# chilir/spotter

Measured on AMD Instinct MI355X. Metric: images/sec RT-DETRv2-R101 640² bs32 at 1/2/4/8 MI355X; p50 /detect latency, higher is better.
Workload: dtype fp32; 1 GPU; RT-DETRv2-r101vd 640x640 batch=32/GPU preprocess+forward+postprocess; model=rtdetr_v2_r101vd, global_batch=32, image_size=640, parallelism=replicas x1

## Files before the change

### include/spotter_hip.h

```cpp
#ifndef SPOTTER_HIP_H
#define SPOTTER_HIP_H

#include <stddef.h>
#include <stdint.h>

#ifdef __cplusplus
extern "C" {
#endif

#define SP_ABI_VERSION 20

enum sp_act { SP_ACT_NONE = 0, SP_ACT_RELU = 1, SP_ACT_SILU = 2, SP_ACT_GELU = 3 };
enum sp_precision { SP_PREC_FP32 = 0, SP_PREC_BF16 = 1, SP_PREC_F32X3 = 2, SP_PREC_F32X2 = 3 };

typedef struct {
  const uint8_t* data;
  int32_t height, width;
  int32_t row_stride;
} sp_image_u8;

typedef struct {
  const float* A; int64_t lda;
  const float* A2; int64_t lda2;
  int32_t N, H, W, Cin;
// ... 72 lines not shown
} sp_conv_plan_info;
int sp_conv_plan(const sp_conv_desc* d, sp_conv_plan_info* out);
int sp_set_plan_batch(int batch, int plan_batch);

int sp_conv3x3_winograd(const sp_conv_desc* d, const uint16_t* wt_wino, int64_t wino_plane_stride, float* work,
                        int64_t work_elems, void* stream);
int sp_winograd_f23_input(const sp_conv_desc* d, float* work, int64_t work_elems, void* stream);
int sp_winograd_f23_gemm(const sp_conv_desc* d, const uint16_t* wt_wino, int64_t wino_plane_stride, float* work,
                         int64_t work_elems, void* stream);
int sp_winograd_f23_output(const sp_conv_desc* d, const float* work, int64_t work_elems, void* stream);
int sp_winograd_f43_input(const sp_conv_desc* d, float* work, int64_t work_elems, void* stream);
int sp_winograd_f43_gemm(const sp_conv_desc* d, const uint16_t* wt_wino, int64_t wino_plane_stride, float* work,
                         int64_t work_elems, void* stream);
int sp_winograd_f43_output(const sp_conv_desc* d, const float* work, int64_t work_elems, void* stream);
typedef struct {
  sp_conv_plan_info gemm;
  int32_t components;
  int32_t in_vw;
  int32_t out_vw;
  int64_t tiles;
} sp_winograd_plan_info;
int sp_winograd_plan(const sp_conv_desc* d, int wm, int64_t wino_plane_stride, int64_t work_elems,
                     sp_winograd_plan_info* out);

int sp_nchw_to_nhwc(const float* x, float* y, int n, int c, int h, int w, void* stream);
int sp_stem_conv3x3s2_nchw(const float* x, const float* wt, const float* scale, const float* shift, float* y,
                           int n, int h, int w, int cout, int act, void* stream);
int sp_stem_conv3x3s2_nchw_bf16(const float* x, const float* wt, const float* scale, const float* shift, uint16_t* y,
                                int n, int h, int w, int cout, int act, void* stream);
int sp_conv3x3_c32_bf16(const uint16_t* x, const uint16_t* w16, const float* scale, const float* shift, uint16_t* y,
                        int n, int h, int w, int cout, int act, void* stream);
int sp_conv3x3_c32(const float* x, const float* wt, const float* scale, const float* shift, float* y, int n, int h,
                   int w, int cout, int act, void* stream);
int sp_conv3x3_c64_bf16(const uint16_t* x, int64_t ldx, const uint16_t* w16, const float* scale, const float* shift,
                        uint16_t* y, int64_t ldy, const uint16_t* res, int64_t ldr, int n, int h, int w, int act,
                        void* stream);
int sp_conv3x3_c64_x3(const float* x, int64_t ldx, const uint16_t* w_planes, int64_t plane_stride, const float* scale,
                      const float* shift, float* y, int64_t ldy, int n, int h, int w, int act, void* stream);
int sp_conv3x3_c32_x3(const float* x, const uint16_t* w_planes, int64_t plane_stride, const float* scale,
                      const float* shift, float* y, int n, int h, int w, int cout, int act, void* stream);
int sp_maxpool3x3s2(const float* x, float* y, int64_t ldy, int n, int h, int w, int c, void* stream);
int sp_maxpool3x3s2_bf16(const uint16_t* x, uint16_t* y, int64_t ldy, int n, int h, int w, int c, void* stream);
int sp_avgpool2x2_ceil(const float* x, float* y, int64_t ldy, int n, int h, int w, int c, void* stream);
int sp_avgpool2x2_ceil_bf16(const uint16_t* x, uint16_t* y, int64_t ldy, int n, int h, int w, int c, void* stream);
int sp_upsample2x_nearest(const float* x, int64_t ldx, float* y, int64_t ldy, int n, int h,
                          int w, int c, void* stream);
// ... 117 lines not shown
```

### spotter_amd/_lib.py

```python
from __future__ import annotations

import ctypes as C
import os
import threading

HERE = os.path.dirname(os.path.abspath(__file__))
LIB_PATH = os.environ.get("SPOTTER_HIP_LIB", os.path.join(HERE, "libspotter_hip.so"))
ABI_VERSION = 20

vp = C.c_void_p
i32 = C.c_int32
i64 = C.c_int64
f32 = C.c_float


class SpImageU8(C.Structure):
    _fields_ = [("data", vp), ("height", i32), ("width", i32), ("row_stride", i32)]


class SpConvDesc(C.Structure):
    _fields_ = [
        ("A", vp), ("lda", i64), ("A2", vp), ("lda2", i64),
        ("N", i32), ("H", i32), ("W", i32), ("Cin", i32),
        ("KH", i32), ("KW", i32), ("stride", i32), ("pad", i32),
# ... 2 lines not shown
        ("scale", vp), ("shift", vp),
        ("row_scale", vp), ("row_period", i32),
        ("res1", vp), ("ldr1", i64),
        ("act", i32),
        ("res2", vp), ("ldr2", i64),
        ("C", vp), ("ldc", i64),
        ("out_rows_per_group", i32), ("out_group_stride", i64),
        ("workspace", vp), ("workspace_elems", i64),
        ("precision", i32), ("Wt_bf16", vp), ("wt_plane_stride", i64),
        ("ln_gamma", vp), ("ln_beta", vp), ("ln_eps", f32),
        ("A_bf16", vp),
        ("C_bf16", vp), ("res1_bf16", vp), ("res2_bf16", vp),
        ("splitk_counters", vp), ("splitk_counters_len", i64),
    ]


class SpConvPlanInfo(C.Structure):
    _fields_ = [(f, i32) for f in ("family", "tile", "planes", "generic", "a_bf16", "fast_1x1", "epilogue", "splits",
                                   "counters")]


class SpWinogradPlanInfo(C.Structure):
    _fields_ = [("gemm", SpConvPlanInfo), ("components", i32), ("in_vw", i32), ("out_vw", i32), ("tiles", i64)]


class SpMsdaDesc(C.Structure):
    _fields_ = [
        ("value", vp), ("ld_value", i64), ("value_col", i32),
        ("off_aw", vp), ("ld_off_aw", i64),
        ("ref", vp),
        ("out", vp), ("ld_out", i64),
        ("B", i32), ("S", i32), ("Q", i32), ("heads", i32), ("head_dim", i32),
        ("levels", i32), ("points", i32),
        ("level_h", i32 * 4), ("level_w", i32 * 4), ("level_start", i32 * 4),
        ("offset_scale", f32),
        ("value_bf16", vp),
    ]


class SpJpegLayout(C.Structure):
    _fields_ = [
        ("width", i32), ("height", i32), ("ncomp", i32), ("color", i32), ("progressive", i32),
        ("max_h", i32), ("max_v", i32), ("h", i32 * 3), ("v", i32 * 3), ("bw", i32 * 3), ("bh", i32 * 3),
        ("block_off", i64 * 3), ("total_blocks", i64), ("plane_off", i64 * 3), ("plane_bytes", i64),
        ("quant", (C.c_uint16 * 64) * 3),
    ]
# ... 47 lines not shown

_SIGS = {
    "sp_abi_version": (i32, []),
    "sp_build_flags": (i32, []),
    "sp_bounds_report": (i64, [C.c_char_p, i64]),
    "sp_last_error": (C.c_char_p, []),
    "sp_device_init": (i32, [i32]),
    "sp_shutdown": (i32, []),
    "sp_preprocess_u8": (i32, [C.POINTER(SpImageU8), i32, i32, i32, vp, vp]),
    "sp_conv2d": (i32, [C.POINTER(SpConvDesc), vp]),
    "sp_set_conv_config": (i32, [i32]),
    "sp_set_splitk_config": (i32, [i32, i32, i32]),
    "sp_set_tuning": (i32, [i32, i32]),
    "sp_set_plan_batch": (i32, [i32, i32]),
    "sp_conv_plan": (i32, [C.POINTER(SpConvDesc), C.POINTER(SpConvPlanInfo)]),
    "sp_winograd_plan": (i32, [C.POINTER(SpConvDesc), i32, i64, i64, C.POINTER(SpWinogradPlanInfo)]),
    "sp_conv3x3_winograd": (i32, [C.POINTER(SpConvDesc), vp, i64, vp, i64, vp]),
    "sp_winograd_f23_input": (i32, [C.POINTER(SpConvDesc), vp, i64, vp]),
    "sp_winograd_f23_gemm": (i32, [C.POINTER(SpConvDesc), vp, i64, vp, i64, vp]),
    "sp_winograd_f23_output": (i32, [C.POINTER(SpConvDesc), vp, i64, vp]),
    "sp_winograd_f43_input": (i32, [C.POINTER(SpConvDesc), vp, i64, vp]),
    "sp_winograd_f43_gemm": (i32, [C.POINTER(SpConvDesc), vp, i64, vp, i64, vp]),
    "sp_winograd_f43_output": (i32, [C.POINTER(SpConvDesc), vp, i64, vp]),
    "sp_nchw_to_nhwc": (i32, [vp, vp, i32, i32, i32, i32, vp]),
    "sp_stem_conv3x3s2_nchw": (i32, [vp, vp, vp, vp, vp, i32, i32, i32, i32, i32, vp]),
    "sp_maxpool3x3s2": (i32, [vp, vp, i64, i32, i32, i32, i32, vp]),
    "sp_avgpool2x2_ceil": (i32, [vp, vp, i64, i32, i32, i32, i32, vp]),
    "sp_maxpool3x3s2_bf16": (i32, [vp, vp, i64, i32, i32, i32, i32, vp]),
    "sp_avgpool2x2_ceil_bf16": (i32, [vp, vp, i64, i32, i32, i32, i32, vp]),
    "sp_stem_conv3x3s2_nchw_bf16": (i32, [vp, vp, vp, vp, vp, i32, i32, i32, i32, i32, vp]),
    "sp_conv3x3_c32_bf16": (i32, [vp, vp, vp, vp, vp, i32, i32, i32, i32, i32, vp]),
    "sp_conv3x3_c32": (i32, [vp, vp, vp, vp, vp, i32, i32, i32, i32, i32, vp]),
    "sp_conv3x3_c64_bf16": (i32, [vp, i64, vp, vp, vp, vp, i64, vp, i64, i32, i32, i32, i32, vp]),
    "sp_conv3x3_c64_x3": (i32, [vp, i64, vp, i64, vp, vp, vp, i64, i32, i32, i32, i32, vp]),
    "sp_conv3x3_c32_x3": (i32, [vp, vp, i64, vp, vp, vp, i32, i32, i32, i32, i32, vp]),
    "sp_upsample2x_nearest": (i32, [vp, i64, vp, i64, i32, i32, i32, i32, vp]),
    "sp_layernorm": (i32, [vp, i64, vp, vp, vp, i64, i32, i32, f32, vp]),
    "sp_layernorm_bf16": (i32, [vp, i64, vp, vp, vp, i64, i32, i32, f32, vp]),
    "sp_attention": (i32, [vp, i64, vp, i64, vp, i64, vp, i64, i32, i32, i32, i32, f32, vp]),
    "sp_attention_bf16": (i32, [vp, i64, vp, i64, vp, i64, vp, i64, i32, i32, i32, i32, f32, vp]),
    "sp_msda": (i32, [C.POINTER(SpMsdaDesc), vp]),
    "sp_topk_rows": (i32, [vp, i64, i32, i32, i32, i32, i32, vp, vp, vp]),
    "sp_rowmax": (i32, [vp, i64, i64, i32, vp, vp]),
    "sp_gather_rows": (i32, [vp, i64, i32, vp, i32, i32, i32, vp, i64, vp]),
    "sp_ref_init": (i32, [vp, i64, vp, vp, i32, i32, vp, vp]),
    "sp_box_refine": (i32, [vp, i64, vp, i32, vp]),
# ... 56 lines not shown
```

### spotter_amd/csrc/winograd.hip

```cpp
#include <cstdlib>
#include "conv_plan.h"
#include "mfma16_common.h"

namespace sp {
namespace {

typedef float v4f __attribute__((ext_vector_type(4)));

__device__ __forceinline__ float4 ld_nt(const float* p) {
  const v4f v = __builtin_nontemporal_load(reinterpret_cast<const v4f*>(p));
  return make_float4(v.x, v.y, v.z, v.w);
}

__global__ __launch_bounds__(256) void wino_in_f23_x2_kernel(const float* __restrict__ x, int64_t lda, int h, int w,
                                                             int c4n, int th, int tw, int64_t nb,
                                                             float* __restrict__ V, int64_t cin) {
  const int tw2 = (tw + 1) / 2;
  const int64_t T = nb * th * tw;
  const int64_t total = nb * th * tw2 * c4n;
  const int64_t plane = T * cin;
  for (int64_t g = blockIdx.x * (int64_t)blockDim.x + threadIdx.x; g < total; g += (int64_t)gridDim.x * blockDim.x) {
    const int64_t t2 = g / c4n;
    const int c = (int)(g - t2 * c4n) * 4;
    const int64_t b = t2 / ((int64_t)th * tw2);
// ... 422 lines not shown
    else
      hipLaunchKernelGGL(wino_out_f43_kernel<2>, dim3(stream_grid(T * d->Cout / 2)), dim3(256), 0,
                         as_stream(stream), work + wino_v_floats(NC, T, d->Cin), T, d->Cout / 2, th, tw, *d, ts, cs);
  }
  return check_launch(what);
}

template <int MT>
int wino_plan_info(const sp_conv_desc* d, int64_t wino_plane_stride, int64_t work_elems, sp_winograd_plan_info* out) {
  WinoPlan w;
  if (int rc = wino_plan<MT>("sp_winograd_plan", d, nullptr, wino_plane_stride, nullptr, work_elems, true, false, &w))
    return rc;
  out->gemm = w.p;
  out->components = (MT + 2) * (MT + 2);
  out->in_vw = w.in_vw;
  out->out_vw = w.out_vw;
  out->tiles = w.T;
  return 0;
}

}
}

extern "C" int sp_winograd_f23_input(const sp_conv_desc* d, float* work, int64_t work_elems, void* stream) {
  return sp::wino_input<2>("sp_winograd_f23_input", d, work, work_elems, stream);
}

extern "C" int sp_winograd_f23_gemm(const sp_conv_desc* d, const uint16_t* wt_wino, int64_t wino_plane_stride,
                                    float* work, int64_t work_elems, void* stream) {
  return sp::wino_gemm<2>("sp_winograd_f23_gemm", d, wt_wino, wino_plane_stride, work, work_elems, stream);
}

extern "C" int sp_winograd_f23_output(const sp_conv_desc* d, const float* work, int64_t work_elems, void* stream) {
  return sp::wino_output<2>("sp_winograd_f23_output", d, work, work_elems, stream);
}

extern "C" int sp_conv3x3_winograd(const sp_conv_desc* d, const uint16_t* wt_wino, int64_t wino_plane_stride,
                                   float* work, int64_t work_elems, void* stream) {
  if (int rc = sp_winograd_f23_input(d, work, work_elems, stream)) return rc;
  if (int rc = sp_winograd_f23_gemm(d, wt_wino, wino_plane_stride, work, work_elems, stream)) return rc;
  return sp_winograd_f23_output(d, work, work_elems, stream);
}

extern "C" int sp_winograd_f43_input(const sp_conv_desc* d, float* work, int64_t work_elems, void* stream) {
  return sp::wino_input<4>("sp_winograd_f43_input", d, work, work_elems, stream);
}
// ... 17 lines not shown
```

### spotter_amd/engine.py

```python
from __future__ import annotations

import math

import numpy as np
import torch

from . import ops
from .config import PRECISIONS, SpotterConfig, check_batch_invariant, check_precision
from .ops import V, view
from .weights import backbone_plan


def _t(a, dev):
    return torch.from_numpy(np.ascontiguousarray(a, dtype=np.float32)).to(dev)


bf16_bits = ops.bf16_bits


ATTN_BF16 = True

_X3_FASTER = {(256, 64, False), (256, 1024, True), (1024, 256, True), (512, 256, True), (256, 512, True),
              (288, 256, True), (4, 256, False)}



def _wkw(wq):
    if wq is None:
        return {}
    if wq.dim() == 2 and wq.shape[0] in (2, 3):
        return {"wt_planes": wq}
    return {"wt16": wq}


class ConvW:
    __slots__ = ("w", "cin", "cout", "k", "scale", "shift", "w16", "host", "wino", "mode", "x3p")

    def __init__(self, w, cin, cout, k, scale, shift, w16=None, host=None, mode="f32"):
        self.w, self.cin, self.cout, self.k, self.scale, self.shift = w, cin, cout, k, scale, shift
        self.w16 = w16
        self.mode = mode
        self.host = host
        self.wino = None
        self.x3p = None


class LinW:
    __slots__ = ("w", "b", "k", "n", "w16", "mode")

    def __init__(self, w, b, k, n, w16=None, mode="f32"):
        self.w, self.b, self.k, self.n = w, b, k, n
        self.w16 = w16
        self.mode = mode


def frozen_bn_affine(p, pre):
    scale = p[pre + ".weight"] * (p[pre + ".running_var"] + np.float32(1e-5)) ** np.float32(-0.5)
    shift = p[pre + ".bias"] - p[pre + ".running_mean"] * scale
    return scale.astype(np.float32), shift.astype(np.float32)


def eval_bn_affine(p, pre, eps=1e-5):
    inv = (p[pre + ".running_var"] + np.float32(eps)) ** np.float32(-0.5)
    scale = p[pre + ".weight"] * inv
    shift = p[pre + ".bias"] - p[pre + ".running_mean"] * scale
    return scale.astype(np.float32), shift.astype(np.float32)

# ... 16 lines not shown
    out = []
    f = np.float32
    for lvl, (h, w) in enumerate(shapes):
        gy, gx = np.meshgrid(np.arange(h, dtype=f), np.arange(w, dtype=f), indexing="ij")
        xy = np.stack([gx, gy], -1) + f(0.5)
        xy[..., 0] /= f(w)
        xy[..., 1] /= f(h)
        wh = np.ones_like(xy) * f(grid_size * 2.0 ** lvl)
        out.append(np.concatenate([xy, wh], -1).reshape(h * w, 4))
    a = np.concatenate(out, 0).astype(f)
    valid = ((a > f(1e-2)) & (a < f(1 - 1e-2))).all(-1)
    lg = np.log(a / (f(1) - a)).astype(f)
    lg[~valid] = np.finfo(f).max
    return lg, valid.astype(f)


class Engine:

    def __init__(self, cfg: SpotterConfig, weights: dict, device: str | torch.device = "cuda",
                 fold_repvgg: bool = True, precision: str = "fp32", fuse_shortcut: bool = True,
                 fuse_ln: bool = False, winograd: str | bool = "auto", wino_m: int = 4,
                 bf16_store: bool | None = None, direct_c32: bool = True,
                 direct_c64_bf16: bool = True, splitk_combine: bool = False, direct_c64_x3: bool = True,
                 direct_c32_x3: bool = False, batch_invariant: int | None = None):
        from ._lib import SP_BUILD_FUSED_LN, lib

        check_precision(precision)
        self.batch_invariant = check_batch_invariant(batch_invariant)
        self.cfg = cfg
        self.fold_repvgg = fold_repvgg
        self.fuse_shortcut = fuse_shortcut
        self.fuse_ln = fuse_ln
        if fuse_ln and PRECISIONS.get(precision, ("", ""))[1] == "bf16":
            raise ValueError(f"fuse_ln=True runs the linears on fp32 weights: not available with precision={precision!r}")
        if fuse_ln and not (lib().sp_build_flags() & SP_BUILD_FUSED_LN):
            raise ValueError("fuse_ln=True needs a diagnostic library with the fused-LayerNorm tiles "
                             "(UNIT=conv_gemm tools/build_diag.sh <name> -DSP_DIAG_KERNELS=1; SPOTTER_HIP_LIB)")
        if winograd is True:
            winograd = "auto"
        if winograd not in (False, None, "auto", "repvgg", "all"):
            raise ValueError("winograd must be False, 'auto', 'repvgg' or 'all'")
        self.winograd = winograd or False
        if wino_m not in (2, 4):
            raise ValueError("wino_m must be 2 (F(2x2,3x3)) or 4 (F(4x4,3x3))")
        self.wino_m = wino_m
        self.precision = precision
        self.act_bb = cfg.hidden_act
        self.act_enc = cfg.activation_function
        self.act_aifi = cfg.encoder_activation_function
        self.act_dec = cfg.decoder_activation_function
        self._conv_mode, self._lin_mode = PRECISIONS[precision]
        self._attn_bf16 = self._lin_mode == "bf16" and ATTN_BF16
        self.bf16_store = (self._conv_mode == "bf16") if bf16_store is None else bool(bf16_store)
        if self.bf16_store and self._conv_mode != "bf16":
            raise ValueError("bf16_store needs a bf16 conv operand mode")
        self.direct_c32 = direct_c32
        self.direct_c64_bf16 = direct_c64_bf16
        self.direct_c64_x3 = direct_c64_x3
        self.direct_c32_x3 = direct_c32_x3
        self.splitk_combine = splitk_combine
        self.splitk_min_rows = 0
        self.add_rows = True
        self.enc_head_bf16 = True
        self.enc_rowmax_fused = True
        self.dev = torch.device(device)
        if self.dev.type != "cuda":
            raise RuntimeError("spotter_amd runs on an MI355X (gfx950) device only")
        idx = self.dev.index if self.dev.index is not None else torch.cuda.current_device()
        self.dev = torch.device("cuda", idx)
        rc = lib().sp_device_init(idx)
        if rc != 0:
            raise RuntimeError(f"sp_device_init: {lib().sp_last_error().decode()}")
        with torch.cuda.device(self.dev):
            self._pack(weights)
        self._B = 1
        self._ws = {}
        self._consts = {}
        self._ctxs = {}
        self._outs = {}
        self.microbatches = None
        self.stagger = 1
# ... 58 lines not shown
        cfg = self.cfg
        bb = "model.backbone.model"
        self.stem = [self._conv(p, f"{bb}.embedder.embedder.{i}.convolution.weight",
                                f"{bb}.embedder.embedder.{i}.normalization", True) for i in range(3)]
        if self.precision == "fp32" and self._conv_mode == "x3" and self.direct_c32_x3:
            for cw in self.stem[1:]:
                if cw.cin == 32 and cw.k == 3 and cw.cout in (32, 64) and cw.mode == "f32":
                    cw.x3p = torch.from_numpy(ops.split_bf16x3_host(cw.host)).to(self.dev)
        self.blocks = []
        for (s, i, lt, cin, cout, st, sc) in backbone_plan(cfg):
            pre = f"{bb}.encoder.stages.{s}.layers.{i}"
            blk = {"s": s, "i": i, "type": lt, "cin": cin, "cout": cout, "stride": st, "sc": sc}
            if sc == "conv":
                blk["short"] = self._conv(p, pre + ".shortcut.convolution.weight", pre + ".shortcut.normalization", True)
            elif sc == "avgconv":
                blk["short"] = self._conv(p, pre + ".shortcut.1.convolution.weight", pre + ".shortcut.1.normalization", True)
            nl = 3 if lt == "bottleneck" else 2
            blk["layers"] = [self._conv(p, f"{pre}.layer.{j}.convolution.weight", f"{pre}.layer.{j}.normalization", True)
                             for j in range(nl)]
            if self.winograd in ("auto", "all"):
                for j, c in enumerate(blk["layers"]):
                    if c.k == 3 and (st == 1 or (lt != "bottleneck" and j == 1)):
                        self._add_wino(c)
            if self.fuse_shortcut and lt == "bottleneck" and (sc == "avgconv" or (sc == "conv" and st == 1)):
                sk = pre + (".shortcut.1" if sc == "avgconv" else ".shortcut")
                blk["fused"] = self._fused_tail(p, f"{pre}.layer.2", sk, cin)
            self.blocks.append(blk)
        self.in_proj = [self._conv(p, f"model.encoder_input_proj.{l}.0.weight", f"model.encoder_input_proj.{l}.1", False)
                        for l in range(len(cfg.encoder_in_channels))]
        a = "model.encoder.aifi.0.layers.0"
        self.aifi = {
            "qk": self._lin(p, a + ".self_attn.q_proj", a + ".self_attn.k_proj"),
            "v": self._lin(p, a + ".self_attn.v_proj"),
            "o": self._lin(p, a + ".self_attn.o_proj"),
            "ln1": self._ln(p, a + ".self_attn_layer_norm"),
            "fc1": self._lin(p, a + ".mlp.fc1"),
            "fc2": self._lin(p, a + ".mlp.fc2"),
            "ln2": self._ln(p, a + ".final_layer_norm"),
        }
        E = "model.encoder"
        nl = len(cfg.encoder_in_channels)
        self.lateral = [self._conv(p, f"{E}.lateral_convs.{i}.conv.weight", f"{E}.lateral_convs.{i}.norm", False)
                        for i in range(nl - 1)]
        self.down = [self._conv(p, f"{E}.downsample_convs.{i}.conv.weight", f"{E}.downsample_convs.{i}.norm", False)
                     for i in range(nl - 1)]
        self.fpn = [self._csp(p, f"{E}.fpn_blocks.{i}") for i in range(nl - 1)]
# ... 113 lines not shown
            return pixels * cin >= self.WINO43_MIN_WORK and (cin >= self.WINO43_MIN_CIN or self.winograd != "auto")
        return pixels >= self.WINO_MIN_PIXELS

    def _cv(self, x: V, n, h, w, cw: ConvW, stride, out: V, act=None, res1=None, res2=None, **kw):
        pad = cw.k // 2
        if (cw.cin == 64 and cw.cout == 64 and cw.k == 3 and stride == 1 and not kw and res2 is None
                and act in ("relu", None) and self._pb(n) * h * w >= self.C64_MIN_PIXELS):
            rows16 = lambda v: v.ld % 8 == 0 and v.off % 8 == 0
            if (self.direct_c64_bf16 and x.is_bf16 and out.is_bf16 and cw.mode == "bf16" and rows16(x)
                    and rows16(out) and (res1 is None or (res1.is_bf16 and rows16(res1)))):
                return ops.conv3x3_c64_bf16(x, cw.w16, cw.scale, cw.shift, out, n, h, w, act=act, res1=res1)
            rows4 = lambda v: not v.is_bf16 and v.ld % 4 == 0 and v.off % 4 == 0
            if self.direct_c64_x3 and cw.mode == "x3" and res1 is None and rows4(x) and rows4(out):
                return ops.conv3x3_c64_x3(x, cw.w16, cw.scale, cw.shift, out, n, h, w, act=act)
        if cw.wino is not None and stride == 1 and not kw and not x.is_bf16 and self._wino_pays(self._pb(n) * h * w, cw.cin):
            wm = self.wino_m
            tiles = n * ((h + wm - 1) // wm) * ((w + wm - 1) // wm)
            work = self._buf("wino_work", ops.wino_work_elems(wm, tiles, cw.cin, cw.cout))
            return ops.conv2d(x, n, h, w, cw.cin, cw.w, cw.cout, 3, 1, 1, out, scale=cw.scale, shift=cw.shift,
                              act=act, res1=res1, res2=res2, wino=(cw.wino, work, wm))
        return ops.conv2d(x, n, h, w, cw.cin, cw.w, cw.cout, cw.k, stride, pad, out, scale=cw.scale,
                          shift=cw.shift, act=act, res1=res1, res2=res2,
                          **self._splitk(), **_wkw(cw.w16), **kw)

    def _lin_op(self, x: V, rows, lw: LinW, out: V, act=None, res1=None, res2=None, a2=None, row_scale=None,
                ln=None):
        if ln is not None and self.fuse_ln:
            if act is not None or res2 is not None:
                raise ValueError("fused LayerNorm epilogue: act / res2 are not implemented")
            if lw.mode == "bf16":
                raise ValueError("fuse_ln runs fp32 weights: not available on a bf16-operand layer")
            return ops.linear(x, rows, lw.k, lw.w, lw.n, out, bias=lw.b, res1=res1, a2=a2, row_scale=row_scale,
                              ln=(ln[0], ln[1], self.cfg.layer_norm_eps))
        if ln is not None:
            tmp = view(self._buf("ln_tmp", rows, lw.n), lw.n)
            ops.linear(x, rows, lw.k, lw.w, lw.n, tmp, bias=lw.b, act=act, res1=res1, res2=res2, a2=a2,
                       row_scale=row_scale, **self._splitk(), **_wkw(lw.w16))
            return ops.layernorm(tmp, *ln, out, rows, lw.n, self.cfg.layer_norm_eps)
        prows = rows if self.batch_invariant is None else rows // self._B * self.batch_invariant
        sk = self._splitk() if prows > self.splitk_min_rows else {}
        return ops.linear(x, rows, lw.k, lw.w, lw.n, out, bias=lw.b, act=act, res1=res1, res2=res2, a2=a2,
                          row_scale=row_scale, **sk, **_wkw(lw.w16))

    def _lin_plus(self, x: V, addend: V | None, rows, lw: LinW, out: V, key: str):
        if addend is None:
            return self._lin_op(x, rows, lw, out)
# ... 77 lines not shown
                self._cv(curv, B, h, w, L[0], 1, view(t1, red), act=self.act_bb)
                self._cv(view(t1, red), B, h, w, L[1], st, V(cat, 0, kc), act=self.act_bb)
                self._cv(V(cat, 0, kc), B, ho, wo, blk["fused"], 1, view(out, cout), act=self.act_bb)
                curv, h, w, c = view(out, cout), ho, wo, cout
                yield
                continue
            if blk["sc"] == "identity":
                res = view(cur, c)
            else:
                src, sh_, sw_ = cur, h, w
                if blk["sc"] == "avgconv":
                    pooled = buf(f"s{s}_pool", B, (h + 1) // 2, (w + 1) // 2, c)
                    ops.avgpool2x2_ceil(cur, pooled, B, h, w, c)
                    src, sh_, sw_ = pooled, (h + 1) // 2, (w + 1) // 2
                sbuf = buf(f"s{s}_sc", B, ho, wo, cout)
                self._cv(view(src, c), B, sh_, sw_, blk["short"], 1 if blk["sc"] == "avgconv" else st, view(sbuf, cout))
                res = view(sbuf, cout)
            out = buf(f"s{s}_out{i % 2}", B, ho, wo, cout)
            if blk["type"] == "bottleneck":
                red = L[0].cout
                t1 = buf(f"s{s}_t1", B, h, w, red)
                t2 = buf(f"s{s}_t2", B, ho, wo, red)
                self._cv(view(cur, c), B, h, w, L[0], 1, view(t1, red), act=self.act_bb)
                self._cv(view(t1, red), B, h, w, L[1], st, view(t2, red), act=self.act_bb)
                self._cv(view(t2, red), B, ho, wo, L[2], 1, view(out, cout), act=self.act_bb, res1=res)
            else:
                t1 = buf(f"s{s}_t1", B, ho, wo, cout)
                self._cv(view(cur, c), B, h, w, L[0], st, view(t1, cout), act=self.act_bb)
                self._cv(view(t1, cout), B, ho, wo, L[1], 1, view(out, cout), act=self.act_bb, res1=res)
            curv, h, w, c = view(out, cout), ho, wo, cout
            yield
        feats.append((curv.t, h, w, c))
        return feats[-3:] if nstage >= 3 else feats

    def _csp_fwd(self, cs, x: V, B, h, w, out: V, tag):
        hid = cs["hid"]
        dt = torch.int16 if self.bf16_store else torch.float32
        c12 = self._buf(f"{tag}_c12", B, h, w, 2 * hid, dtype=dt)
        self._cv(x, B, h, w, cs["c12"], 1, view(c12, 2 * hid), act=self.act_enc)
        h2 = V(c12, hid, 2 * hid)
        cur = V(c12, 0, 2 * hid)
        t = None if self.fold_repvgg else self._buf(f"{tag}_t", B, h, w, hid, dtype=dt)
        final_to_out = cs["c3"] is None
        for b, (k3, k1) in enumerate(cs["reps"]):
            last = b == len(cs["reps"]) - 1
            if last and final_to_out:
                dst = out
            else:
# ... 268 lines not shown
```

### spotter_amd/ops.py

```python
from __future__ import annotations

import ctypes as C
from dataclasses import dataclass

import numpy as np
import torch

from ._lib import SpConvDesc, SpImageU8, SpMsdaDesc, call

ACT = {None: 0, "none": 0, "relu": 1, "silu": 2, "gelu": 3}
PREC_BY_PLANES = {1: 1, 3: 2, 2: 3}
PREC_TAG = ("f32", "bf16", "x3", "x2")

_hook = None


def set_launch_hook(hook):
    global _hook
    _hook = hook


def _launch(kind: str, name: str, args, flops: int = 0, nbytes: int = 0, shape=None):
    if _hook is None:
        call(name, *args)
# ... 196 lines not shown
             (m, cout, "out"))]


def wino_launch(stages, only=None):
    for st in stages:
        if only is None or st[1].endswith("_" + only):
            _launch(*st)


def wino_plan(desc, wm: int, plane_stride: int | None = None, work_elems: int | None = None) -> dict:
    from ._lib import SpConvPlanInfo, SpWinogradPlanInfo, call

    nc = (wm + 2) ** 2
    tiles = desc.N * ((desc.H + wm - 1) // wm) * ((desc.W + wm - 1) // wm)
    ps = nc * desc.Cout * desc.Cin if plane_stride is None else plane_stride
    we = wino_work_elems(wm, tiles, desc.Cin, desc.Cout) if work_elems is None else work_elems
    info = SpWinogradPlanInfo()
    call("sp_winograd_plan", C.byref(desc), int(wm), int(ps), int(we), C.byref(info))
    out = {f: getattr(info, f) for f in ("components", "in_vw", "out_vw", "tiles")}
    out["gemm"] = {f: getattr(info.gemm, f) for f, _ in SpConvPlanInfo._fields_}
    return out


def linear(x: V, rows: int, k: int, wt: torch.Tensor, n: int, out: V, *, bias=None, act=None,
           res1: V | None = None, res2: V | None = None, a2: V | None = None, row_scale=None,
           scale=None, workspace=None, wt16=None, wt_planes=None, ln=None, counters=None):
    return conv2d(x, 1, 1, rows, k, wt, n, 1, 1, 0, out, scale=scale, shift=bias, act=act, res1=res1,
                  res2=res2, a2=a2, row_scale=row_scale, workspace=workspace, wt16=wt16, wt_planes=wt_planes,
                  ln=ln, counters=counters)


def bf16_bits(a) -> np.ndarray:
    u = np.ascontiguousarray(a, dtype=np.float32).view(np.uint32).astype(np.uint64)
    return ((u + 0x7FFF + ((u >> 16) & 1)) >> 16).astype(np.uint16)


def _bf16_float(bits: np.ndarray) -> np.ndarray:
    return (bits.astype(np.uint32) << 16).view(np.float32)


def split_bf16x3_host(w) -> np.ndarray:
    w = np.ascontiguousarray(w, dtype=np.float32).reshape(-1)
    hi = bf16_bits(w)
    r1 = w - _bf16_float(hi)
    mid = bf16_bits(r1)
    lo = bf16_bits(r1 - _bf16_float(mid))
# ... 378 lines not shown
```

Measured before the change: 797.9 images/sec.

## Fuse Winograd F(4,3) output transform with following 1x1 expand conv

Adds a HIP kernel that runs the Winograd F(4x4,3x3) output transform, BN and ReLU of the bottleneck's 3x3 conv and writes the result as bf16x3 split planes into LDS. The following 1x1 expand conv then runs as an MFMA GEMM on that LDS tile, with residual add and activation applied in the epilogue. This skips the intermediate t2 write and re-read and one kernel launch, for stride-1 bottlenecks above a pixel threshold. Expand weights are pre-packed into fragment order at load time. The cost is one block per CU with large LDS use, which may limit occupancy.

Result: faster. 826.0 images/sec, median of 6 (+3.5%).

```diff
diff --git a/include/spotter_hip.h b/include/spotter_hip.h
--- a/include/spotter_hip.h
+++ b/include/spotter_hip.h
@@ -118,6 +118,19 @@
 } sp_winograd_plan_info;
 int sp_winograd_plan(const sp_conv_desc* d, int wm, int64_t wino_plane_stride, int64_t work_elems,
                      sp_winograd_plan_info* out);
+
+typedef struct {
+  sp_conv_plan_info expand;
+  int32_t fused;
+  int32_t reserved;
+  int64_t tiles;
+  int64_t units;
+} sp_winograd_expand_plan_info;
+int sp_winograd_f43_expand(const sp_conv_desc* conv2, const float* work, int64_t work_elems,
+                           const sp_conv_desc* expand, const uint16_t* expand_frag, int64_t frag_elems,
+                           int64_t min_pixels, void* stream);
+int sp_winograd_expand_plan(const sp_conv_desc* conv2, int64_t work_elems, const sp_conv_desc* expand, int has_frag,
+                            int64_t min_pixels, sp_winograd_expand_plan_info* out);
 
 int sp_nchw_to_nhwc(const float* x, float* y, int n, int c, int h, int w, void* stream);
 int sp_stem_conv3x3s2_nchw(const float* x, const float* wt, const float* scale, const float* shift, float* y,
diff --git a/spotter_amd/_lib.py b/spotter_amd/_lib.py
--- a/spotter_amd/_lib.py
+++ b/spotter_amd/_lib.py
@@ -48,6 +48,10 @@
 
 class SpWinogradPlanInfo(C.Structure):
     _fields_ = [("gemm", SpConvPlanInfo), ("components", i32), ("in_vw", i32), ("out_vw", i32), ("tiles", i64)]
+
+
+class SpWinogradExpandPlanInfo(C.Structure):
+    _fields_ = [("expand", SpConvPlanInfo), ("fused", i32), ("reserved", i32), ("tiles", i64), ("units", i64)]
 
 
 class SpMsdaDesc(C.Structure):
@@ -141,6 +145,9 @@
     "sp_winograd_f43_input": (i32, [C.POINTER(SpConvDesc), vp, i64, vp]),
     "sp_winograd_f43_gemm": (i32, [C.POINTER(SpConvDesc), vp, i64, vp, i64, vp]),
     "sp_winograd_f43_output": (i32, [C.POINTER(SpConvDesc), vp, i64, vp]),
+    "sp_winograd_f43_expand": (i32, [C.POINTER(SpConvDesc), vp, i64, C.POINTER(SpConvDesc), vp, i64, i64, vp]),
+    "sp_winograd_expand_plan": (i32, [C.POINTER(SpConvDesc), i64, C.POINTER(SpConvDesc), i32, i64,
+                                      C.POINTER(SpWinogradExpandPlanInfo)]),
     "sp_nchw_to_nhwc": (i32, [vp, vp, i32, i32, i32, i32, vp]),
     "sp_stem_conv3x3s2_nchw": (i32, [vp, vp, vp, vp, vp, i32, i32, i32, i32, i32, vp]),
     "sp_maxpool3x3s2": (i32, [vp, vp, i64, i32, i32, i32, i32, vp]),
diff --git a/spotter_amd/csrc/wino_expand.hip b/spotter_amd/csrc/wino_expand.hip
--- /dev/null
+++ b/spotter_amd/csrc/wino_expand.hip
@@ -0,0 +1,350 @@
+#include <type_traits>
+
+#include "conv_plan.h"
+#include "mfma16_common.h"
+
+namespace sp {
+
+int wino43_geometry(const char* what, const sp_conv_desc* d, const float* work, int64_t work_elems, bool ptrs,
+                    int* th, int* tw, int64_t* T);
+
+namespace {
+
+constexpr int WX_PX = 96;
+constexpr int WX_NCHUNK = 256;
+
+struct WxArgs {
+  const float* M;
+  int64_t T, units;
+  int th, tw, H, W;
+  const float* sc2;
+  const float* sh2;
+  int act2;
+  const uint4* wf;
+  const float* scale;
+  const float* shift;
+  int act;
+  const float* res1;
+  int64_t ldr1;
+  float* C;
+  int64_t ldc;
+  int Cout;
+  int wbytes;
+  int rbytes, cbytes;
+};
+
+typedef float v4f __attribute__((ext_vector_type(4)));
+
+constexpr float kAT[4][6] = {{1.f, 1.f, 1.f, 1.f, 1.f, 0.f},
+                             {0.f, -1.f, 1.f, 0.5f, -2.f, 0.f},
+                             {0.f, 1.f, 1.f, 0.25f, 4.f, 0.f},
+                             {0.f, -1.f, 1.f, 0.125f, -8.f, 1.f}};
+
+__device__ __forceinline__ int wx_swz(int row, int chunk) { return chunk ^ (row & 15); }
+
+template <int K>
+__global__ __launch_bounds__(512, 1) void wino_expand_kernel(const WxArgs a) {
+  constexpr int CPP = K / 8;
+  constexpr int NS = K / 16;
+  constexpr int C4 = K / 4;
+  constexpr int PLANE = WX_PX * CPP;
+  static_assert(CPP % 16 == 0, "the swizzle permutes 16 chunks");
+  __shared__ uint4 lds[3 * PLANE];
+  static_assert(sizeof(lds) == (K == 256 ? 147456 : 73728), "static LDS bytes");
+  const int tid = threadIdx.x, lane = tid & 63;
+  const int wave = __builtin_amdgcn_readfirstlane(tid >> 6);
+  const int r = lane & 31, h = lane >> 5;
+
+  const int64_t u0 = a.units * blockIdx.x / gridDim.x, u1 = a.units * (blockIdx.x + 1) / gridDim.x;
+  const int nrun = (int)(u1 - u0);
+  const int ntile = (nrun + 2) / 3;
+  const int64_t mplane = a.T * K;
+  const int tht = a.th * a.tw;
+  const int ldr = (int)a.ldr1, ldc = (int)a.ldc;
+  const __amdgpu_buffer_rsrc_t rrs =
+      __builtin_amdgcn_make_buffer_rsrc(const_cast<float*>(a.res1), 0, a.rbytes, 0x00020000);
+  const __amdgpu_buffer_rsrc_t crs = __builtin_amdgcn_make_buffer_rsrc(a.C, 0, a.cbytes, 0x00020000);
+  const __amdgpu_buffer_rsrc_t wrs =
+      __builtin_amdgcn_make_buffer_rsrc(const_cast<uint4*>(a.wf), 0, a.wbytes, 0x00020000);
+  const int vres = (h * a.W * ldr + r) * 4, vout = (h * a.W * ldc + r) * 4;
+
+  for (int tile = 0; tile < ntile; ++tile) {
+    const int64_t ub = u0 + (int64_t)nrun * tile / ntile;
+    const int nu = (int)(u0 + (int64_t)nrun * (tile + 1) / ntile - ub);
+    __syncthreads();
+    for (int it = tid; it < 2 * nu * C4; it += 512) {
+      const int tt = it / C4, c = (it - tt * C4) * 4;
+      const int64_t t = 2 * ub + tt;
+      v4f s[4][6];
+#pragma unroll
+      for (int p = 0; p < 4; ++p)
+#pragma unroll
+        for (int bb = 0; bb < 6; ++bb) s[p][bb] = v4f(0.f);
+      const bool tok = t < a.T;
+      if (tok) {
+        const float* src = a.M + t * K + c;
+        SP_BCHECK(35 * mplane + t * K + c + 3, 36 * mplane);
+        v4f mr[2][6];
+#pragma unroll
+        for (int bb = 0; bb < 6; ++bb)
+          mr[0][bb] = __builtin_nontemporal_load(reinterpret_cast<const v4f*>(src + bb * mplane));
+#pragma unroll
+        for (int aa = 0; aa < 6; ++aa) {
+          if (aa + 1 < 6) {
+#pragma unroll
+            for (int bb = 0; bb < 6; ++bb)
+              mr[(aa + 1) & 1][bb] =
+                  __builtin_nontemporal_load(reinterpret_cast<const v4f*>(src + ((aa + 1) * 6 + bb) * mplane));
+          }
+#pragma unroll
+          for (int p = 0; p < 4; ++p)
+            if (kAT[p][aa] != 0.f)
+#pragma unroll
+              for (int bb = 0; bb < 6; ++bb)
+                s[p][bb] = __builtin_elementwise_fma(v4f(kAT[p][aa]), mr[aa & 1][bb], s[p][bb]);
+          __builtin_amdgcn_sched_barrier(0);
+        }
+      }
+      const v4f sc = a.sc2 ? *reinterpret_cast<const v4f*>(a.sc2 + c) : v4f(1.f);
+      const v4f sh = a.sh2 ? *reinterpret_cast<const v4f*>(a.sh2 + c) : v4f(0.f);
+      uint2* dst = reinterpret_cast<uint2*>(lds);
+#pragma unroll
+      for (int p = 0; p < 4; ++p)
+#pragma unroll
+        for (int qq = 0; qq < 4; ++qq) {
+          v4f y = v4f(0.f);
+#pragma unroll
+          for (int bb = 0; bb < 6; ++bb)
+            if (kAT[qq][bb] != 0.f) y = __builtin_elementwise_fma(v4f(kAT[qq][bb]), s[p][bb], y);
+          y = __builtin_elementwise_fma(y, sc, sh);
+#pragma unroll
+          for (int e = 0; e < 4; ++e) y[e] = tok ? (a.act2 ? fmaxf(y[e], 0.f) : y[e]) : 0.f;
+          bf16x8 pl[3];
+          split_frag_pk<3>(make_float4(y[0], y[1], y[2], y[3]), make_float4(0.f, 0.f, 0.f, 0.f), pl);
+          const int row = tt * 16 + p * 4 + qq;
+          const int pos = (row * CPP + wx_swz(row, c >> 3)) * 2 + ((c >> 2) & 1);
+#pragma unroll
+          for (int q = 0; q < 3; ++q) {
+            const uint4 v = __builtin_bit_cast(uint4, pl[q]);
+            dst[q * PLANE * 2 + pos] = make_uint2(v.x, v.y);
+          }
+        }
+    }
+    __syncthreads();
+
+    int pix0[3][2], hrem[3][2], wrem[3][2];
+#pragma unroll
+    for (int u = 0; u < 3; ++u)
+#pragma unroll
+      for (int tt = 0; tt < 2; ++tt) {
+        const int t = 2 * ((int)ub + u) + tt;
+        const bool ok = u < nu && t < (int)a.T;
+        const int tc = ok ? t : 0;
+        const int b = tc / tht, rem = tc - b * tht;
+        const int ty = rem / a.tw, tx = rem - ty * a.tw;
+        pix0[u][tt] = (b * a.H + 4 * ty) * a.W + 4 * tx;
+        hrem[u][tt] = ok ? a.H - 4 * ty : 0;
+        wrem[u][tt] = a.W - 4 * tx;
+      }
+
+    auto gemm = [&](auto nuc) {
+      constexpr int NU = decltype(nuc)::value;
+      for (int n0 = wave * 32; n0 < a.Cout; n0 += WX_NCHUNK) {
+        const int wb = (n0 >> 5) * (NS * 3 * 1024);
+        SP_BCHECK(wb + (NS * 3 - 1) * 1024 + lane * 16 + 15, a.wbytes);
+        int p0[NU][2], hr[NU][2], wr[NU][2];
+#pragma unroll
+        for (int u = 0; u < NU; ++u)
+#pragma unroll
+          for (int tt = 0; tt < 2; ++tt) {
+            p0[u][tt] = pix0[u][tt];
+            hr[u][tt] = hrem[u][tt];
+            wr[u][tt] = wrem[u][tt];
+            asm volatile("" : "+s"(p0[u][tt]), "+s"(hr[u][tt]), "+s"(wr[u][tt]));
+          }
+        f32x16 acc[NU];
+        zero_acc(acc);
+        bf16x8 wfr[3][3];
+        bf16x8 xa[2][3];
+        float res[NU][16];
+        auto load_w = [&](int s) {
+#pragma unroll
+          for (int q = 0; q < 3; ++q)
+            wfr[s % 3][q] = __builtin_bit_cast(
+                bf16x8, __builtin_amdgcn_raw_buffer_load_b128(wrs, lane * 16, wb + (s * 3 + q) * 1024, 0));
+        };
+        int x0 = (r * CPP + wx_swz(r, h)) * 16;
+        asm volatile("" : "+v"(x0));
+        auto load_x = [&](int i) {
+          const int s = i / NU, u = i - s * NU;
+          const char* base = reinterpret_cast<const char*>(lds) + ((x0 ^ (s << 5)) + u * (32 * CPP * 16));
+#pragma unroll
+          for (int q = 0; q < 3; ++q) xa[i & 1][q] = *reinterpret_cast<const bf16x8*>(base + q * (PLANE * 16));
+        };
+        load_w(0);
+        load_w(1);
+        load_x(0);
+#pragma unroll
+        for (int u = 0; u < NU; ++u)
+#pragma unroll
+          for (int q = 0; q < 16; ++q) res[u][q] = 0.f;
+#pragma unroll
+        for (int s = 0; s < NS; ++s) {
+          if (s + 2 < NS) load_w(s + 2);
+          if (s == NS / 2 && a.res1) {
+#pragma unroll
+            for (int u = 0; u < NU; ++u)
+#pragma unroll
+              for (int q = 0; q < 16; ++q) {
+                const int tt = q >> 3, pp = (q >> 2) & 1, qq = q & 3;
+                const bool ok = 2 * pp + h < hr[u][tt] && qq < wr[u][tt];
+                const int so = (p0[u][tt] + 2 * pp * a.W + qq) * (ldr * 4) + n0 * 4;
+                res[u][q] = __builtin_bit_cast(
+                    float, __builtin_amdgcn_raw_buffer_load_b32(rrs, ok ? vres : 0x7ffffffc, so, 0));
+              }
+          }
+#pragma unroll
+          for (int u = 0; u < NU; ++u) {
+            const int i = s * NU + u;
+            if (i + 1 < NS * NU) load_x(i + 1);
+            acc[u] = mfma_planes<3>(xa[i & 1], wfr[s % 3], acc[u]);
+            __builtin_amdgcn_sched_barrier(0);
+          }
+          __builtin_amdgcn_sched_barrier(0);
+        }
+        const float sc = a.scale ? a.scale[n0 + r] : 1.0f;
+        const float sh = a.shift ? a.shift[n0 + r] : 0.0f;
+#pragma unroll
+        for (int u = 0; u < NU; ++u)
+#pragma unroll
+          for (int q = 0; q < 16; ++q) {
+            const int tt = q >> 3, pp = (q >> 2) & 1, qq = q & 3;
+            const bool ok = 2 * pp + h < hr[u][tt] && qq < wr[u][tt];
+            const int so = (p0[u][tt] + 2 * pp * a.W + qq) * (ldc * 4) + n0 * 4;
+            if (ok) SP_BCHECK((int64_t)so + vout, a.cbytes);
+            float v = fmaf(acc[u][q], sc, sh);
+            if (a.res1) v += res[u][q];
+            v = a.act ? fmaxf(v, 0.f) : v;
+            __builtin_amdgcn_raw_buffer_store_b32(__builtin_bit_cast(uint32_t, v), crs, ok ? vout : 0x7ffffffc, so, 0);
+          }
+      }
+    };
+    if (nu == 3) gemm(std::integral_constant<int, 3>{});
+    else if (nu == 2) gemm(std::integral_constant<int, 2>{});
+    else gemm(std::integral_constant<int, 1>{});
+  }
+}
+
+constexpr bool glds_is_m16(int id) {
+  switch (id) {
+#define SP_WX_M16(id, WM, WN, TM, TN, NS, BK, M16, OCC, AB) \
+  case id:                                                  \
+    return M16;
+    SP_GLDS_CONFIGS(SP_WX_M16)
+#undef SP_WX_M16
+    default:
+      return false;
+  }
+}
+
+constexpr bool wx_k_built(int k) { return k == 256 || k == 128; }
+
+struct WxPlan {
+  int th, tw;
+  int64_t T;
+  ConvArgs ea;
+  ConvPlan ep;
+  int fused;
+};
+
+int wx_plan(const char* what, const sp_conv_desc* c2, const float* work, int64_t work_elems, bool ptrs,
+            const sp_conv_desc* ex, bool has_frag, const uint16_t* frag, int64_t frag_elems, int64_t min_pixels,
+            WxPlan* w) {
+  SP_ARG_CHECK(c2 != nullptr && ex != nullptr, "%s: null descriptor", what);
+  if (int rc = wino43_geometry(what, c2, work, work_elems, ptrs, &w->th, &w->tw, &w->T)) return rc;
+  int planes;
+  if (conv_args(ex, conv_overrides(), &w->ea, &planes) || plan_conv(w->ea, planes, conv_overrides(), &w->ep)) return -1;
+  SP_ARG_CHECK(ex->KH == 1 && ex->KW == 1 && ex->stride == 1 && ex->pad == 0 && ex->N == c2->N && ex->H == c2->H &&
+                   ex->W == c2->W && ex->Cin == c2->Cout && ex->A == c2->C && ex->lda == c2->ldc,
+               "%s: the expand must be a 1x1 stride-1 conv reading conv2's output rows (A = conv2's C, lda = its ldc, "
+               "Cin = its Cout, the same N, H, W)", what);
+  SP_ARG_CHECK(!has_frag || (frag_elems >= (int64_t)3 * ex->Cout * ex->Cin &&
+                             (!ptrs || (frag && (reinterpret_cast<uintptr_t>(frag) & 15) == 0))),
+               "%s: fragment-order planes: %lld < 3*Cout*K elements, or null / not 16-byte aligned", what,
+               (long long)frag_elems);
+  const ConvPlan& p = w->ep;
+  w->fused = has_frag && p.family == SP_CONV_GLDS && p.planes == 3 && p.splits == 1 && !p.a_bf16 &&
+             !glds_is_m16(p.tile) && wx_k_built(ex->Cin) && ex->Cout % 32 == 0 && !ex->res2 && !ex->res2_bf16 &&
+             !ex->res1_bf16 && !ex->C_bf16 && !ex->A2 && !ex->row_scale && ex->out_rows_per_group == 0 &&
+             (int64_t)ex->Cout * ex->Cin * 6 < (int64_t(1) << 31) && !ex->ln_gamma && !c2->res1 && !c2->res2 && ex->act <= SP_ACT_RELU && c2->act <= SP_ACT_RELU &&
+             ((w->ea.M - 1) * ex->ldc + ex->Cout) * 4 < (int64_t(1) << 31) - 4 &&
+             (!ex->res1 || ((w->ea.M - 1) * ex->ldr1 + ex->Cout) * 4 < (int64_t(1) << 31) - 4) &&
+             w->ea.Mp >= min_pixels;
+  return 0;
+}
+
+template <int K>
+int wx_launch(const WxArgs& a, hipStream_t s) {
+  const int64_t cap = g_num_cus > 0 ? g_num_cus : 1;
+  const unsigned grid = (unsigned)(a.units < cap ? a.units : cap);
+  hipLaunchKernelGGL(wino_expand_kernel<K>, dim3(grid), dim3(512), 0, s, a);
+  return check_launch("sp_winograd_f43_expand");
+}
+
+}
+}
+
+extern "C" int sp_winograd_f43_expand(const sp_conv_desc* conv2, const float* work, int64_t work_elems,
+                                      const sp_conv_desc* expand, const uint16_t* expand_frag, int64_t frag_elems,
+                                      int64_t min_pixels, void* stream) {
+  using namespace sp;
+  const char* what = "sp_winograd_f43_expand";
+  WxPlan w;
+  if (int rc = wx_plan(what, conv2, work, work_elems, true, expand, expand_frag != nullptr, expand_frag, frag_elems,
+                       min_pixels, &w))
+    return rc;
+  if (!w.fused) {
+    if (int rc = sp_winograd_f43_output(conv2, work, work_elems, stream)) return rc;
+    return launch_plan(w.ea, w.ep, as_stream(stream));
+  }
+  WxArgs a;
+  a.M = work + (int64_t)36 * w.T * conv2->Cin;
+  a.T = w.T;
+  a.units = (w.T + 1) / 2;
+  a.th = w.th;
+  a.tw = w.tw;
+  a.H = conv2->H;
+  a.W = conv2->W;
+  a.sc2 = conv2->scale;
+  a.sh2 = conv2->shift;
+  a.act2 = conv2->act;
+  a.wf = reinterpret_cast<const uint4*>(expand_frag);
+  a.scale = expand->scale;
+  a.shift = expand->shift;
+  a.act = expand->act;
+  a.res1 = expand->res1;
+  a.ldr1 = expand->ldr1;
+  a.C = expand->C;
+  a.ldc = expand->ldc;
+  a.Cout = expand->Cout;
+  a.wbytes = 3 * expand->Cout * expand->Cin * 2;
+  a.cbytes = (int)(((w.ea.M - 1) * expand->ldc + expand->Cout) * 4);
+  a.rbytes = expand->res1 ? (int)(((w.ea.M - 1) * expand->ldr1 + expand->Cout) * 4) : 0;
+  return expand->Cin == 256 ? wx_launch<256>(a, as_stream(stream)) : wx_launch<128>(a, as_stream(stream));
+}
+
+extern "C" int sp_winograd_expand_plan(const sp_conv_desc* conv2, int64_t work_elems, const sp_conv_desc* expand,
+                                       int has_frag, int64_t min_pixels, sp_winograd_expand_plan_info* out) {
+  using namespace sp;
+  SP_ARG_CHECK(out != nullptr, "sp_winograd_expand_plan: null out");
+  WxPlan w;
+  if (int rc = wx_plan("sp_winograd_expand_plan", conv2, nullptr, work_elems, false, expand, has_frag != 0, nullptr,
+                       expand ? (int64_t)3 * expand->Cout * expand->Cin : 0, min_pixels, &w))
+    return rc;
+  out->expand = w.ep;
+  out->fused = w.fused;
+  out->reserved = 0;
+  out->tiles = w.T;
+  out->units = (w.T + 1) / 2;
+  return 0;
+}
diff --git a/spotter_amd/csrc/winograd.hip b/spotter_amd/csrc/winograd.hip
--- a/spotter_amd/csrc/winograd.hip
+++ b/spotter_amd/csrc/winograd.hip
@@ -468,6 +468,13 @@
 }
 }
 
+namespace sp {
+int wino43_geometry(const char* what, const sp_conv_desc* d, const float* work, int64_t work_elems, bool ptrs,
+                    int* th, int* tw, int64_t* T) {
+  return wino_check<4>(what, d, nullptr, 0, work, work_elems, false, ptrs, th, tw, T);
+}
+}
+
 extern "C" int sp_winograd_f23_input(const sp_conv_desc* d, float* work, int64_t work_elems, void* stream) {
   return sp::wino_input<2>("sp_winograd_f23_input", d, work, work_elems, stream);
 }
diff --git a/spotter_amd/engine.py b/spotter_amd/engine.py
--- a/spotter_amd/engine.py
+++ b/spotter_amd/engine.py
@@ -34,7 +34,7 @@
 
 
 class ConvW:
-    __slots__ = ("w", "cin", "cout", "k", "scale", "shift", "w16", "host", "wino", "mode", "x3p")
+    __slots__ = ("w", "cin", "cout", "k", "scale", "shift", "w16", "host", "wino", "mode", "x3p", "xfrag")
 
     def __init__(self, w, cin, cout, k, scale, shift, w16=None, host=None, mode="f32"):
         self.w, self.cin, self.cout, self.k, self.scale, self.shift = w, cin, cout, k, scale, shift
@@ -43,6 +43,7 @@
         self.host = host
         self.wino = None
         self.x3p = None
+        self.xfrag = None
 
 
 class LinW:
@@ -105,7 +106,7 @@
                  fuse_ln: bool = False, winograd: str | bool = "auto", wino_m: int = 4,
                  bf16_store: bool | None = None, direct_c32: bool = True,
                  direct_c64_bf16: bool = True, splitk_combine: bool = False, direct_c64_x3: bool = True,
-                 direct_c32_x3: bool = False, batch_invariant: int | None = None):
+                 direct_c32_x3: bool = False, batch_invariant: int | None = None, wino_expand: bool = True):
         from ._lib import SP_BUILD_FUSED_LN, lib
 
         check_precision(precision)
@@ -140,6 +141,7 @@
         self.direct_c32 = direct_c32
         self.direct_c64_bf16 = direct_c64_bf16
         self.direct_c64_x3 = direct_c64_x3
+        self.wino_expand = wino_expand
         self.direct_c32_x3 = direct_c32_x3
         self.splitk_combine = splitk_combine
         self.splitk_min_rows = 0
@@ -244,6 +246,11 @@
                 for j, c in enumerate(blk["layers"]):
                     if c.k == 3 and (st == 1 or (lt != "bottleneck" and j == 1)):
                         self._add_wino(c)
+            c2, c3 = (blk["layers"][1], blk["layers"][2]) if lt == "bottleneck" else (None, None)
+            if (self.wino_expand and c2 is not None and c2.wino is not None and self.wino_m == 4 and st == 1
+                    and c3.mode == "x3" and c3.k == 1 and c3.cin in (128, 256) and c3.cout % 32 == 0):
+                c3.xfrag = torch.from_numpy(ops.pack_expand_frag_host(ops.split_bf16x3_host(c3.host), c3.cout,
+                                                                      c3.cin)).to(self.dev)
             if self.fuse_shortcut and lt == "bottleneck" and (sc == "avgconv" or (sc == "conv" and st == 1)):
                 sk = pre + (".shortcut.1" if sc == "avgconv" else ".shortcut")
                 blk["fused"] = self._fused_tail(p, f"{pre}.layer.2", sk, cin)
@@ -403,6 +410,25 @@
         return ops.conv2d(x, n, h, w, cw.cin, cw.w, cw.cout, cw.k, stride, pad, out, scale=cw.scale,
                           shift=cw.shift, act=act, res1=res1, res2=res2,
                           **self._splitk(), **_wkw(cw.w16), **kw)
+
+    WINO_EXPAND_MIN_PIXELS = 3200
+
+    def _cv_wino_expand(self, x: V, n, h, w, c2: ConvW, stride, t2: V, c3: ConvW, out: V, res: V) -> bool:
+        if not (self.wino_expand and c3.xfrag is not None and c2.wino is not None and self.wino_m == 4 and stride == 1
+                and not x.is_bf16 and self.act_bb in ("relu", None)
+                and self._wino_pays(self._pb(n) * h * w, c2.cin)):
+            return False
+        tiles = n * ((h + 3) // 4) * ((w + 3) // 4)
+        work = self._buf("wino_work", ops.wino_work_elems(4, tiles, c2.cin, c2.cout))
+        d2, _ = ops.conv_desc(x, n, h, w, c2.cin, c2.w, c2.cout, 3, 1, 1, t2, scale=c2.scale, shift=c2.shift,
+                              act=self.act_bb)
+        stages = ops.wino_desc(d2, (c2.wino, work, 4))
+        ops.wino_launch(stages, only="input")
+        ops.wino_launch(stages, only="gemm")
+        de, hook_args = ops.conv_desc(t2, n, h, w, c3.cin, c3.w, c3.cout, 1, 1, 0, out, scale=c3.scale, shift=c3.shift,
+                                      act=self.act_bb, res1=res, **self._splitk(), **_wkw(c3.w16))
+        ops.wino_expand(stages, d2, work, de, hook_args, c3.xfrag, self.WINO_EXPAND_MIN_PIXELS)
+        return True
 
     def _lin_op(self, x: V, rows, lw: LinW, out: V, act=None, res1=None, res2=None, a2=None, row_scale=None,
                 ln=None):
@@ -526,8 +552,9 @@
                 t1 = buf(f"s{s}_t1", B, h, w, red)
                 t2 = buf(f"s{s}_t2", B, ho, wo, red)
                 self._cv(view(cur, c), B, h, w, L[0], 1, view(t1, red), act=self.act_bb)
-                self._cv(view(t1, red), B, h, w, L[1], st, view(t2, red), act=self.act_bb)
-                self._cv(view(t2, red), B, ho, wo, L[2], 1, view(out, cout), act=self.act_bb, res1=res)
+                if not self._cv_wino_expand(view(t1, red), B, h, w, L[1], st, view(t2, red), L[2], view(out, cout), res):
+                    self._cv(view(t1, red), B, h, w, L[1], st, view(t2, red), act=self.act_bb)
+                    self._cv(view(t2, red), B, ho, wo, L[2], 1, view(out, cout), act=self.act_bb, res1=res)
             else:
                 t1 = buf(f"s{s}_t1", B, ho, wo, cout)
                 self._cv(view(cur, c), B, h, w, L[0], st, view(t1, cout), act=self.act_bb)
diff --git a/spotter_amd/ops.py b/spotter_amd/ops.py
--- a/spotter_amd/ops.py
+++ b/spotter_amd/ops.py
@@ -242,6 +242,45 @@
     return out
 
 
+def pack_expand_frag_host(planes, cout: int, k: int) -> np.ndarray:
+    p = np.asarray(planes)
+    if p.shape != (3, cout * k) or cout % 32 or k % 16:
+        raise ValueError(f"expand fragments: planes {p.shape} are not [3, {cout}*{k}] with Cout % 32 == 0, K % 16 == 0")
+    p = p.reshape(3, cout // 32, 32, k // 16, 2, 8)
+    return np.ascontiguousarray(p.transpose(1, 3, 0, 4, 2, 5)).reshape(-1)
+
+
+def pack_expand_frag(planes: torch.Tensor, cout: int, k: int) -> torch.Tensor:
+    return torch.from_numpy(pack_expand_frag_host(planes.detach().cpu().numpy(), cout, k)).to(planes.device)
+
+
+def wino_expand_plan(d2, work_elems: int, de, has_frag: bool = True, min_pixels: int = 0) -> dict:
+    from ._lib import SpConvPlanInfo, SpWinogradExpandPlanInfo, call
+
+    info = SpWinogradExpandPlanInfo()
+    call("sp_winograd_expand_plan", C.byref(d2), int(work_elems), C.byref(de), int(bool(has_frag)), int(min_pixels),
+         C.byref(info))
+    return {"fused": info.fused, "tiles": info.tiles, "units": info.units,
+            "expand": {f: getattr(info.expand, f) for f, _ in SpConvPlanInfo._fields_}}
+
+
+def wino_expand(stages, d2, work: torch.Tensor, de, hook_args, frag: torch.Tensor | None, min_pixels: int = 0):
+    if frag is not None and (frag.dtype != torch.int16 or not frag.is_cuda or not frag.is_contiguous()
+                             or frag.numel() != 3 * de.Cout * de.Cin):
+        raise ValueError("wino_expand: fragment planes must be a contiguous int16 CUDA tensor of 3*Cout*K elements")
+    fused = bool(wino_expand_plan(d2, work.numel(), de, frag is not None, min_pixels)["fused"])
+    if not fused:
+        wino_launch(stages, only="output")
+        conv_launch(de, hook_args)
+        return False
+    m, cout, k = de.N * de.Ho * de.Wo, de.Cout, de.Cin
+    nbytes = 4 * (36 * d2.N * ((d2.H + 3) // 4) * ((d2.W + 3) // 4) * k + m * cout * (1 + bool(de.res1))) + 2 * frag.numel()
+    _launch("conv", "sp_winograd_f43_expand",
+            (C.byref(d2), work.data_ptr(), work.numel(), C.byref(de), frag.data_ptr(), frag.numel(), int(min_pixels),
+             stream()), 2 * m * cout * k, nbytes, (m, cout, k, 1, 1, "x3", "epi:res" if de.res1 else "epi:bn"))
+    return True
+
+
 def linear(x: V, rows: int, k: int, wt: torch.Tensor, n: int, out: V, *, bias=None, act=None,
            res1: V | None = None, res2: V | None = None, a2: V | None = None, row_scale=None,
            scale=None, workspace=None, wt16=None, wt_planes=None, ln=None, counters=None):
```
